# antopio26/quadruped-gym

Hardware: AMD Instinct MI355X
Metric: env_steps_per_sec (higher is better)
Workload: dtype f32

## Files before the change

### quadruped-gym_amd/csrc/qg_kernel_link.hip

```cpp
#define QGK_LINK_ENVS 4
#include "qg_po_dev.h"

typedef const __attribute__((address_space(1))) char *lk_gcbytes;
typedef __attribute__((address_space(1))) char *lk_gbytes;
template <class T> DEV T lk_ld(const T *base, unsigned byte_off) { return *(const __attribute__((address_space(1))) T *)((lk_gcbytes)base + byte_off); }
template <class T> DEV void lk_st(T *base, unsigned byte_off, T v) { *(__attribute__((address_space(1))) T *)((lk_gbytes)base + byte_off) = v; }

template <int CTRL> DEV float dpp_any(float x) {
    return __builtin_bit_cast(float, __builtin_amdgcn_mov_dpp(__builtin_bit_cast(int, x), CTRL, 0xF, 0xF, true));
}
DEV float env_sum(float x) {
#pragma clang fp contract(off)
    x += dpp_any<0xB1>(x);
    x += dpp_any<0x4E>(x);
    x += dpp_any<0x141>(x);
    x += dpp_any<0x140>(x);
    return x;
}
DEV V3 env_sum(V3 a) { return v3(env_sum(a.x), env_sum(a.y), env_sum(a.z)); }
#define QG_T_HM(d, s, bm) "v_add_f32_dpp %[" d "], %[" s "], %[" s "] row_half_mirror row_mask:0xf bank_mask:" bm "\n\t"
#define QG_T_ROR(d, s, bm) "v_add_f32_dpp %[" d "], %[" s "], %[" s "] row_ror:8 row_mask:0xf bank_mask:" bm "\n\t"
#define QG_T_QP(d, qp) "v_add_f32_dpp %[" d "], %[" d "], %[" d "] quad_perm:" qp " row_mask:0xf bank_mask:0xf\n\t"
#define QG_T_L1(g) QG_T_HM("a" g, "a" g, "0x5") QG_T_HM("c" g, "c" g, "0x5") QG_T_HM("a" g, "b" g, "0xa") QG_T_HM("c" g, "d" g, "0xa")
#define QG_T_L2(g) QG_T_ROR("a" g, "a" g, "0x3") QG_T_ROR("a" g, "c" g, "0xc")
#define QG_T_Q1(g) QG_T_QP("a" g, "[1,0,3,2]")
#define QG_T_Q2(g) QG_T_QP("a" g, "[2,3,0,1]")
#define QG_T_OUT(g, v) [a##g] "+v"(v[4 * g]), [c##g] "+v"(v[4 * g + 2])
#define QG_T_IN(g, v) [b##g] "v"(v[4 * g + 1]), [d##g] "v"(v[4 * g + 3])
DEV void env_sum_banked16(float (&v)[16]) {
    asm("s_nop 1\n\t" QG_T_L1("0") QG_T_L1("1") QG_T_L1("2") QG_T_L1("3") QG_T_L2("0") QG_T_L2("1") QG_T_L2("2") QG_T_L2("3")
        QG_T_Q1("0") QG_T_Q1("1") QG_T_Q1("2") QG_T_Q1("3") QG_T_Q2("0") QG_T_Q2("1") QG_T_Q2("2") QG_T_Q2("3") "s_nop 1"
        : QG_T_OUT(0, v), QG_T_OUT(1, v), QG_T_OUT(2, v), QG_T_OUT(3, v)
        : QG_T_IN(0, v), QG_T_IN(1, v), QG_T_IN(2, v), QG_T_IN(3, v));
}
DEV void env_sum_banked12(float (&v)[12]) {
    asm("s_nop 1\n\t" QG_T_L1("0") QG_T_L1("1") QG_T_L1("2") QG_T_L2("0") QG_T_L2("1") QG_T_L2("2")
        QG_T_Q1("0") QG_T_Q1("1") QG_T_Q1("2") QG_T_Q2("0") QG_T_Q2("1") QG_T_Q2("2") "s_nop 1"
        : QG_T_OUT(0, v), QG_T_OUT(1, v), QG_T_OUT(2, v)
        : QG_T_IN(0, v), QG_T_IN(1, v), QG_T_IN(2, v));
}
template <int K> DEV float banked_sum(float r) { return dpp_any<0x150 + 4 * K>(r); }
DEV float leg_suffix(float x) {
#pragma clang fp contract(off)
    x += dpp_any<0xF9>(x);
    x += dpp_any<0xFE>(x);
    return x;
}
#define QG_Z_FM(i) "v_fmac_f32_dpp %[z" i "], %[z" i "], %[c] quad_perm:[1,1,1,1] row_mask:0xf bank_mask:0xf\n\t"
DEV float leg_bcast0(float x) { return dpp_any<0x00>(x); }
DEV float leg_bcast1(float x) { return dpp_any<0x55>(x); }
DEV float leg_bcast2(float x) { return dpp_any<0xAA>(x); }

DEV float leg_prefix(float x) {
#pragma clang fp contract(off)
    x += dpp_any<0xD3>(x);
    x += dpp_any<0x4F>(x);
    return x;
}
DEV V3 leg_prefix(V3 a) { return v3(leg_prefix(a.x), leg_prefix(a.y), leg_prefix(a.z)); }

struct LinkRegs {
    float mass, ipos[3], inertia[6], cp[QGK_CP_LINK][3];
    f2 cp2[QGK_CP_LINK / 2][3];
    float lo, hi, damping, armature, kp, kv, gear, force_lo, force_hi, act_decay;
    float cpF[3];
    float ml;
    float fb[8];
};
struct HingeLane { float q, qd, act, u, sn, cs; };
struct KXfrcLink { KWrench w; V3 c0; };

DEV float sel3(int r, float a, float b, float c) { return r == 0 ? a : (r == 1 ? b : c); }
DEV V3 sel3(int r, V3 a, V3 b, V3 c) { return v3(sel3(r, a.x, b.x, c.x), sel3(r, a.y, b.y, c.y), sel3(r, a.z, b.z, c.z)); }

template <bool BAKED, bool DYN = false>
DEV void substep_link(const KModel &C, float cm, float sm, int r, bool lead_env, BaseState &B, HingeLane &J, const LinkRegs &K,
                      bool want_sensors, float *__restrict__ row, int kleg, float &zaxis_z, const KDyn &D = KDyn{}, bool xon = false,
                      const KXfrcLink &X = KXfrcLink{}) {
    using namespace pk3;
    const float h = C.h;
    const BaseCtx bc = pk3::base_prelude_unit<BAKED>(C, B);
    const V3 nb = bc.n;
    if (want_sensors) {
        zaxis_z = bc.cz.z;
        if (r < 3) row[3 * kleg + r] = J.q;
        if (lead_env) {
            row[15] = B.wb.x; row[16] = B.wb.y; row[17] = B.wb.z;
            row[18] = B.pw.x; row[19] = B.pw.y; row[20] = B.pw.z;
            row[21] = B.vw.x; row[22] = B.vw.y; row[23] = B.vw.z;
            row[24] = bc.cx.x; row[25] = bc.cx.y; row[26] = bc.cx.z;
            row[27] = bc.cz.x; row[28] = bc.cz.y; row[29] = bc.cz.z;
            row[30] = bc.vb.x; row[31] = bc.vb.y; row[32] = bc.vb.z;
        }
    }
    const int rr = r < 2 ? r : 2;
    const float snj[3] = {leg_bcast0(J.sn), leg_bcast1(J.sn), leg_bcast2(J.sn)};
    const float csj[3] = {leg_bcast0(J.cs), leg_bcast1(J.cs), leg_bcast2(J.cs)};
    Fr E[3];
    V3 p[3];
    SV S[3];
    {
        Fr Ep = {v3(BAKED ? cm : 1.f, BAKED ? sm : 0.f, 0.f), v3(BAKED ? -sm : 0.f, BAKED ? cm : 1.f, 0.f), v3(0.f, 0.f, 1.f)};
        V3 pp = v3(0.f, 0.f, 0.f);
#pragma unroll
        for (int i = 0; i < 3; ++i) {
            const KLink &L = link_of<BAKED>(C, kleg, i);
            const float sn = snj[i], cs = csj[i];
            p[i] = pp + rot(Ep, ld3(L.pos));
            V3 tx = fma3(L.Q[0], Ep.ex, fma3(L.Q[3], Ep.ey, L.Q[6] * Ep.ez));
            V3 ty = fma3(L.Q[1], Ep.ex, fma3(L.Q[4], Ep.ey, L.Q[7] * Ep.ez));
            V3 tz = fma3(L.Q[2], Ep.ex, fma3(L.Q[5], Ep.ey, L.Q[8] * Ep.ez));
            E[i].ex = fma3(cs, tx, sn * ty);
            E[i].ey = fma3(cs, ty, (-sn) * tx);
            E[i].ez = tz;
            S[i].a = E[i].ez;
            S[i].l = cross(p[i], E[i].ez);
            Ep = E[i]; pp = p[i];
        }
    }
    const Fr Ep = {sel3(rr, E[0].ex, E[1].ex, E[2].ex), sel3(rr, E[0].ey, E[1].ey, E[2].ey), sel3(rr, E[0].ez, E[1].ez, E[2].ez)};
    const V3 pp = sel3(rr, p[0], p[1], p[2]);
    const SV So = {Ep.ez, cross(pp, Ep.ez)};
    SV vp, ap;
    {
        const float qdm = K.ml * J.qd;
        const SV Sq = {qdm * So.a, qdm * So.l};
        vp.a = leg_prefix(Sq.a) + bc.V0.a;
        vp.l = leg_prefix(Sq.l) + bc.V0.l;
        const V3 ca = cross(vp.a, Sq.a);
        const V3 cl = cross_add(vp.l, Sq.a, cross(vp.a, Sq.l));
        ap.a = leg_prefix(ca) + bc.A0.a;
        ap.l = leg_prefix(cl) + bc.A0.l;
    }
    Rigid Bi;
    Bi.m = K.mass;
    V3 cl;
    {
        const Fr &E = Ep;
        V3 c = pp + rot(E, v3(K.ipos[0], K.ipos[1], K.ipos[2]));
        cl = c;
        Bi.h = Bi.m * c;
        V3 ux = fma3(K.inertia[0], E.ex, fma3(K.inertia[3], E.ey, K.inertia[4] * E.ez));
        V3 uy = fma3(K.inertia[3], E.ex, fma3(K.inertia[1], E.ey, K.inertia[5] * E.ez));
        V3 uz = fma3(K.inertia[4], E.ex, fma3(K.inertia[5], E.ey, K.inertia[2] * E.ez));
        float hc = dot(Bi.h, c);
        const f2 uxp = {ux.x, ux.y}, uyp = {uy.x, uy.y}, uzp = {uz.x, uz.y}, hp = {Bi.h.x, Bi.h.y}, cp2 = {c.x, c.y};
        const f2 d2 = __builtin_elementwise_fma(uxp, f2{E.ex.x, E.ex.y}, __builtin_elementwise_fma(uyp, f2{E.ey.x, E.ey.y}, uzp * f2{E.ez.x, E.ez.y}))
                      + f2{hc, hc} - hp * cp2;
        const f2 o2 = __builtin_elementwise_fma(uxp, f2{E.ex.z, E.ex.z}, __builtin_elementwise_fma(uyp, f2{E.ey.z, E.ey.z}, uzp * f2{E.ez.z, E.ez.z}))
                      - hp * f2{c.z, c.z};
        Bi.I.xx = d2.x; Bi.I.yy = d2.y; Bi.I.xz = o2.x; Bi.I.yz = o2.y;
        Bi.I.zz = fmaf(ux.z, E.ex.z, fmaf(uy.z, E.ey.z, uz.z * E.ez.z)) + hc - Bi.h.z * c.z;
        Bi.I.xy = fmaf(ux.x, E.ex.y, fmaf(uy.x, E.ey.y, uz.x * E.ez.y)) - Bi.h.x * c.y;
    }
    SV f;
    {
        SV Iv = mul(Bi, vp), Ia = mul(Bi, ap);
        f.a = cross_add(vp.l, Iv.l, cross_add(vp.a, Iv.a, Ia.a));
        f.l = cross_add(vp.a, Iv.l, Ia.l);
    }
    Sym6 A = sym6_of(Bi);
    {
        const float zo = B.pw.z + dot(nb, pp);
        V3 nl = rotT(Ep, nb);
        float wsum = 0.f;
        V3 s = v3(0.f, 0.f, 0.f);
        const float zb = C.contact_margin - zo;
        if constexpr (BAKED) {
            static_assert(QGK_CP_LINK % 2 == 0, "sample points are taken in pairs");
            f2 w2 = {0.f, 0.f};
            V3T<f2> s2 = v3<f2>(w2, w2, w2);
            const V3T<f2> nl2 = v3<f2>(f2{nl.x, nl.x}, f2{nl.y, nl.y}, f2{nl.z, nl.z});
            const f2 zb2 = {zb, zb};
#pragma unroll
            for (int i = 0; i < QGK_CP_LINK / 2; ++i) contact_point(v3<f2>(K.cp2[i][0], K.cp2[i][1], K.cp2[i][2]), nl2, zb2, w2, s2);
            wsum = w2.x + w2.y;
            s = v3(opaque(s2.x.x + s2.x.y), opaque(s2.y.x + s2.y.y), s2.z.x + s2.z.y);
        } else {
#pragma unroll
            for (int i = 0; i < QGK_CP_LINK; ++i) contact_point(v3(K.cp[i][0], K.cp[i][1], K.cp[i][2]), nl, zb, wsum, s);
        }
        wsum *= K.ml;
        SV fe;
        ContactDampT<float> cd;
        if constexpr (DYN) pk3::contact_eval(wsum, s, Ep, pp, nb, vp, D.kc, D.cc, C.contact_inv_ramp, D.mu, h, fe, cd);
        else pk3::contact_eval(wsum, s, Ep, pp, nb, vp, C.contact_k, C.contact_c, C.contact_inv_ramp, C.contact_mu, h, fe, cd);
        f.a = f.a - fe.a;
        f.l = f.l - fe.l;
        if constexpr (BAKED) pk3::add_contact_damping<true>(A, cd.mc, cd.w, cd.P, nb, Bi.h);
        else pk3::add_contact_damping(A, cd.mc, cd.w, cd.P, nb);
    }
    SV xw = {};
    if constexpr (DYN) {
        if (xon) {
            xw = xfrc_spatial(bc, X.w, r < 3 ? cl : X.c0);
            f.a = fma3(-K.ml, xw.a, f.a);
            f.l = fma3(-K.ml, xw.l, f.l);
        }
    }
    float wsumF = 0.f;
    V3 sF = v3(0.f, 0.f, 0.f);
    contact_point(v3(K.cpF[0], K.cpF[1], K.cpF[2]), nb, C.contact_margin - B.pw.z, wsumF, sF);
    wsumF *= K.ml; sF = K.ml * sF;
    Sym6 Ic;
    SV fc;
    Ic.AA.xx = leg_suffix(A.AA.xx); Ic.AA.yy = leg_suffix(A.AA.yy); Ic.AA.zz = leg_suffix(A.AA.zz);
    Ic.AA.xy = leg_suffix(A.AA.xy); Ic.AA.xz = leg_suffix(A.AA.xz); Ic.AA.yz = leg_suffix(A.AA.yz);
    Ic.AL.r0 = v3(leg_suffix(A.AL.r0.x), leg_suffix(A.AL.r0.y), leg_suffix(A.AL.r0.z));
    Ic.AL.r1 = v3(leg_suffix(A.AL.r1.x), leg_suffix(A.AL.r1.y), leg_suffix(A.AL.r1.z));
    Ic.AL.r2 = v3(leg_suffix(A.AL.r2.x), leg_suffix(A.AL.r2.y), leg_suffix(A.AL.r2.z));
    Ic.LL.xx = leg_suffix(A.LL.xx); Ic.LL.yy = leg_suffix(A.LL.yy); Ic.LL.zz = leg_suffix(A.LL.zz);
    Ic.LL.xy = leg_suffix(A.LL.xy); Ic.LL.xz = leg_suffix(A.LL.xz); Ic.LL.yz = leg_suffix(A.LL.yz);
    fc.a = v3(leg_suffix(f.a.x), leg_suffix(f.a.y), leg_suffix(f.a.z));
    fc.l = v3(leg_suffix(f.l.x), leg_suffix(f.l.y), leg_suffix(f.l.z));
    const SV F = mul(Ic, So);
    const float Hc0 = dot(S[0], F), Hc1 = dot(S[1], F);
    const float Hown = dot(So, F);
    const float tb = dot(So, fc);
    float Hd_o, b_o;
    {
        const float q = J.q, qd = J.qd, act = J.act;
        float force = K.kp * (act - K.gear * q) - (K.kv * K.gear) * qd;
        const bool clamped = force <= K.force_lo || force >= K.force_hi;
        force = fminf(fmaxf(force, K.force_lo), K.force_hi);
        float dimp = K.damping + (clamped ? 0.f : K.kv * K.gear * K.gear);
        float tau = K.gear * force - K.damping * qd;
        const float below = K.lo - q, above = q - K.hi;
        const float pen = fmaxf(fmaxf(below, above), 0.f);
        const float bl = C.limit_b * fminf(pen * C.limit_inv_ramp, 1.f);
        const float sg = below > above ? 1.f : -1.f;
        const float sqd = sg * qd;
        const float spring = C.limit_k * pen;
        const float tq = spring - bl * sqd;
        const bool leaving = tq < 0.f;
        tau = fmaf(sg, fmaxf(tq, 0.f), tau);
        dimp = dimp + (leaving ? spring * rcp(sqd) : bl);
        Hd_o = Hown + K.armature + h * dimp;
        b_o = tau - tb;
    }
    const float H00 = leg_bcast0(Hd_o), H01 = leg_bcast1(Hc0), H11 = leg_bcast1(Hd_o);
    const float H02 = leg_bcast2(Hc0), H12 = leg_bcast2(Hc1), H22 = leg_bcast2(Hd_o);
    const float b0 = leg_bcast0(b_o), b1 = leg_bcast1(b_o), b2 = leg_bcast2(b_o);
    const float id0 = rcp(H00);
    const float l10 = H01 * id0, l20 = H02 * id0;
    const float d1 = fmaf(-l10, H01, H11), id1 = rcp(d1);
    const float t21 = fmaf(-l20, H01, H12);
    const float l21 = t21 * id1;
    const float d2 = fmaf(-l21, t21, fmaf(-l20, H02, H22)), id2 = rcp(d2);
    const float y0 = b0, y1 = fmaf(-l10, y0, b1), y2 = fmaf(-l21, y1, fmaf(-l20, y0, b2));
    float z[6] = {F.a.x, F.a.y, F.a.z, F.l.x, F.l.y, F.l.z};
    {
        const float nc0 = r == 1 ? -l10 : (r == 2 ? -l20 : 0.f), nc1 = r == 2 ? -l21 : 0.f;
#pragma unroll
        for (int i = 0; i < 6; ++i) z[i] = fmaf(leg_bcast0(z[i]), nc0, z[i]);
        if constexpr (BAKED) {
            asm("s_nop 1\n\t" QG_Z_FM("0") QG_Z_FM("1") QG_Z_FM("2") QG_Z_FM("3") QG_Z_FM("4") QG_Z_FM("5")
                : [z0] "+v"(z[0]), [z1] "+v"(z[1]), [z2] "+v"(z[2]), [z3] "+v"(z[3]), [z4] "+v"(z[4]), [z5] "+v"(z[5])
                : [c] "v"(nc1));
        } else {
#pragma unroll
            for (int i = 0; i < 6; ++i) z[i] = fmaf(leg_bcast1(z[i]), nc1, z[i]);
        }
    }
    const float idr = sel3(rr, id0, id1, id2), yr = sel3(rr, y0, y1, y2);
    const f2 P = {z[0], z[1]}, L = {z[3], z[4]}, Z = {z[2], z[5]};
    const f2 idr2 = {idr, idr};
    const f2 WP = idr2 * P, WL = idr2 * L, WZ = idr2 * Z;
    Sym6 Cn;
    {
        const f2 Zlo = {Z.x, Z.x}, Zhi = {Z.y, Z.y};
        const f2 WPlo = {WP.x, WP.x}, WPhi = {WP.y, WP.y}, WZlo = {WZ.x, WZ.x};
        const f2 aa0 = __builtin_elementwise_fma(-WP, P, f2{A.AA.xx, A.AA.yy});
        const f2 aa1 = __builtin_elementwise_fma(-WP, Zlo, f2{A.AA.xz, A.AA.yz});
        Cn.AA.xx = aa0.x; Cn.AA.yy = aa0.y; Cn.AA.xz = aa1.x; Cn.AA.yz = aa1.y;
        Cn.AA.xy = fmaf(-WP.x, P.y, A.AA.xy); Cn.AA.zz = fmaf(-WZ.x, Z.x, A.AA.zz);
        const f2 c0 = __builtin_elementwise_fma(-WPlo, L, f2{A.AL.r0.x, A.AL.r0.y});
        const f2 c1 = __builtin_elementwise_fma(-WPhi, L, f2{A.AL.r1.x, A.AL.r1.y});
        const f2 c2 = __builtin_elementwise_fma(-WZlo, L, f2{A.AL.r2.x, A.AL.r2.y});
        const f2 c3 = __builtin_elementwise_fma(-WP, Zhi, f2{A.AL.r0.z, A.AL.r1.z});
        Cn.AL.r0 = v3(c0.x, c0.y, c3.x);
        Cn.AL.r1 = v3(c1.x, c1.y, c3.y);
        Cn.AL.r2 = v3(c2.x, c2.y, fmaf(-WZ.x, Z.y, A.AL.r2.z));
        const f2 l0 = __builtin_elementwise_fma(-WL, L, f2{A.LL.xx, A.LL.yy});
        const f2 l1 = __builtin_elementwise_fma(-WL, Zhi, f2{A.LL.xz, A.LL.yz});
        Cn.LL.xx = l0.x; Cn.LL.yy = l0.y; Cn.LL.xz = l1.x; Cn.LL.yz = l1.y;
        Cn.LL.xy = fmaf(-WL.x, L.y, A.LL.xy); Cn.LL.zz = fmaf(-WZ.y, Z.y, A.LL.zz);
    }
    if constexpr (DYN) {
        if (xon) {
            f.a = fma3(K.ml - 1.f, xw.a, f.a);
            f.l = fma3(K.ml - 1.f, xw.l, f.l);
        }
    }
    const f2 nyr = {-yr, -yr};
    const f2 rh0 = __builtin_elementwise_fma(nyr, WP, f2{-f.a.x, -f.a.y}), rh1 = __builtin_elementwise_fma(nyr, WL, f2{-f.l.x, -f.l.y}),
             rh2 = BAKED ? __builtin_elementwise_fma(nyr, WZ, -f2{f.a.z, f.l.z})
                         : __builtin_elementwise_fma(nyr, WZ, f2{-f.a.z, -f.l.z});
    SV rhn = {v3(rh0.x, rh0.y, rh2.x), v3(rh1.x, rh1.y, rh2.y)};
    float x6[6];
    {
        SV p0;
        Sym6 Ic0;
        pk3::frame_body_pk<DYN>(C, bc, h, p0, Ic0, D);
        if constexpr (BAKED) {
            Ic0.AA.xx = K.fb[0]; Ic0.AA.yy = K.fb[1]; Ic0.AA.zz = K.fb[2]; Ic0.LL.xx = K.fb[3]; Ic0.LL.yy = K.fb[4]; Ic0.LL.zz = K.fb[5];
            Ic0.AL.r0.y = K.fb[6]; Ic0.AL.r1.x = K.fb[7];
        }
        float t16[16] = {Cn.AA.xx, Cn.AA.yy, Cn.AA.zz, Cn.AA.xy, Cn.AA.xz, Cn.AA.yz, Cn.AL.r0.x, Cn.AL.r0.y,
                         Cn.AL.r0.z, Cn.AL.r1.x, Cn.AL.r1.y, Cn.AL.r1.z, Cn.AL.r2.x, Cn.AL.r2.y, Cn.AL.r2.z, wsumF};
        float t12[12] = {Cn.LL.xx, Cn.LL.yy, Cn.LL.zz, Cn.LL.xy, Cn.LL.xz, Cn.LL.yz, rhn.a.x, rhn.a.y, rhn.a.z, rhn.l.x, rhn.l.y, rhn.l.z};
        env_sum_banked16(t16);
        env_sum_banked12(t12);
        Ic0.AA.xx += banked_sum<0>(t16[0]); Ic0.AA.yy += banked_sum<1>(t16[0]); Ic0.AA.zz += banked_sum<2>(t16[0]); Ic0.AA.xy += banked_sum<3>(t16[0]);
        Ic0.AA.xz += banked_sum<0>(t16[4]); Ic0.AA.yz += banked_sum<1>(t16[4]); Ic0.AL.r0.x += banked_sum<2>(t16[4]); Ic0.AL.r0.y += banked_sum<3>(t16[4]);
        Ic0.AL.r0.z += banked_sum<0>(t16[8]); Ic0.AL.r1.x += banked_sum<1>(t16[8]); Ic0.AL.r1.y += banked_sum<2>(t16[8]); Ic0.AL.r1.z += banked_sum<3>(t16[8]);
        Ic0.AL.r2.x += banked_sum<0>(t16[12]); Ic0.AL.r2.y += banked_sum<1>(t16[12]); Ic0.AL.r2.z += banked_sum<2>(t16[12]);
        wsumF = banked_sum<3>(t16[12]);
        Ic0.LL.xx += banked_sum<0>(t12[0]); Ic0.LL.yy += banked_sum<1>(t12[0]); Ic0.LL.zz += banked_sum<2>(t12[0]); Ic0.LL.xy += banked_sum<3>(t12[0]);
        Ic0.LL.xz += banked_sum<0>(t12[4]); Ic0.LL.yz += banked_sum<1>(t12[4]);
        SV b = {v3(banked_sum<2>(t12[4]) - p0.a.x, banked_sum<3>(t12[4]) - p0.a.y, banked_sum<0>(t12[8]) - p0.a.z),
                v3(banked_sum<1>(t12[8]) - p0.l.x, banked_sum<2>(t12[8]) - p0.l.y, banked_sum<3>(t12[8]) - p0.l.z)};
        if (__any(wsumF > 0.f)) {
            sF = env_sum(sF);
            Fr E0 = {v3(1.f, 0.f, 0.f), v3(0.f, 1.f, 0.f), v3(0.f, 0.f, 1.f)};
            SV fe;
            if constexpr (DYN) contact_finish(wsumF, sF, E0, v3(0.f, 0.f, 0.f), bc.n, bc.V0, D.kc, D.cc, C.contact_inv_ramp, D.mu, h, fe, Ic0);
            else contact_finish(wsumF, sF, E0, v3(0.f, 0.f, 0.f), bc.n, bc.V0, C.contact_k, C.contact_c, C.contact_inv_ramp, C.contact_mu, h, fe, Ic0);
            b.a = b.a + fe.a;
            b.l = b.l + fe.l;
        }
        pk3::base_solve(Ic0, b, x6);
    }
    const V3 wdot = v3(x6[0], x6[1], x6[2]);
    const V3 acl = v3(x6[3], x6[4], x6[5]);
    if (want_sensors && lead_env) {
        row[12] = acl.x - bc.gb.x; row[13] = acl.y - bc.gb.y; row[14] = acl.z - bc.gb.z;
    }
    {
        const float g_o = fmaf(F.a.x, x6[0], fmaf(F.a.y, x6[1], fmaf(F.a.z, x6[2], fmaf(F.l.x, x6[3], fmaf(F.l.y, x6[4], F.l.z * x6[5])))));
        const float r0 = b0 - leg_bcast0(g_o), r1 = b1 - leg_bcast1(g_o), r2 = b2 - leg_bcast2(g_o);
        const float yy0 = r0, yy1 = fmaf(-l10, yy0, r1), yy2 = fmaf(-l21, yy1, fmaf(-l20, yy0, r2));
        const float qdd2 = yy2 * id2;
        const float qdd1 = fmaf(-l21, qdd2, yy1 * id1);
        const float qdd0 = fmaf(-l20, qdd2, fmaf(-l10, qdd1, yy0 * id0));
        J.qd = fmaf(h, sel3(rr, qdd0, qdd1, qdd2), J.qd);
        J.q = fmaf(h, J.qd, J.q);
        hinge_advance(h * J.qd, J.sn, J.cs);
        J.act = fmaf(J.u - J.act, K.act_decay, J.act);
    }
    pk3::base_integrate_unit<BAKED>(bc, h, wdot, acl, B);
}

#define QGK_LINK_WAVES 4
template <bool WALK = false, bool PO = false, bool BAKED = true, bool HELP = false, bool DYN = false>
__global__ __launch_bounds__(QGK_WAVE * QGK_LINK_WAVES * (HELP ? 2 : 1), 1) void qg_step_kernel_link(const KModel *__restrict__ Mp, const KTask *__restrict__ T, KStepArgs P,
                                                                                  const typename WalkArgT<WALK>::type WK,
                                                                                  const typename PoArgT<PO>::type PK) {
    static_assert(WALK || !PO, "the observation pack rides on the walking task layer");
    static_assert(WALK || !HELP, "the helper waves carry the walking task layer's estimator");
    static_assert(!DYN || (!BAKED && !HELP), "per-env dynamics: the table-driven variants");
    static_assert(QGK_LINK_ENVS * QGK_LINK_WAVES == QG_PO_ENVS && QGK_WAVE * QGK_LINK_WAVES == QG_PO_THREADS, "workgroup layout of qg_po_dev.h");
    __shared__ float tile_all[QGK_LINK_WAVES][QGK_LINK_ENVS * 35];
    __shared__ KModel smodel;
    QG_STAGE_MODEL(C, BAKED, smodel, Mp, QGK_WAVE * QGK_LINK_WAVES * (HELP ? 2 : 1));
    QG_TASK_REGS(Tk, T);
// ... 302 lines not shown
```

### quadruped-gym_amd/csrc/qg_kernels.hip

```cpp
#include <hip/hip_runtime.h>
#include <stdint.h>

#include "qg_device.h"
#include "qg_model_baked.h"
#include "qg_step_shell.h"

#define DEV __device__ __forceinline__
#define QG_STR2(x) #x
#define QG_STR(x) QG_STR2(x)

static __device__ const KModel QG_BAKED_MODEL = {QG_BAKED_FLOATS};
template <bool BAKED> DEV const KModel &table(const KModel *__restrict__ M) {
    if constexpr (BAKED) return QG_BAKED_MODEL; else return *M;
}
template <bool BAKED> DEV const KLink &link_of(const KModel &C, int k, int i) { return C.link[BAKED ? i : 3 * k + i]; }

typedef float f2 __attribute__((ext_vector_type(2)));
typedef int i2 __attribute__((ext_vector_type(2)));

DEV float fma_(float a, float b, float c) { return fmaf(a, b, c); }
DEV f2 fma_(f2 a, f2 b, f2 c) { return __builtin_elementwise_fma(a, b, c); }
DEV float max_(float a, float b) { return fmaxf(a, b); }
DEV f2 max_(f2 a, f2 b) { f2 r = {fmaxf(a.x, b.x), fmaxf(a.y, b.y)}; return r; }
DEV float min_(float a, float b) { return fminf(a, b); }
// ... 5 lines not shown
DEV float sqrt_(float x) { return __builtin_amdgcn_sqrtf(x); }
DEV f2 sqrt_(f2 x) { f2 r = {__builtin_amdgcn_sqrtf(x.x), __builtin_amdgcn_sqrtf(x.y)}; return r; }
DEV float sel(bool m, float a, float b) { return m ? a : b; }
DEV f2 sel(i2 m, f2 a, f2 b) { f2 r = {m.x ? a.x : b.x, m.y ? a.y : b.y}; return r; }
DEV bool m_and(bool a, bool b) { return a && b; }
DEV i2 m_and(i2 a, i2 b) { return a & b; }
DEV bool m_or(bool a, bool b) { return a || b; }
DEV i2 m_or(i2 a, i2 b) { return a | b; }
DEV bool m_not(bool a) { return !a; }
DEV i2 m_not(i2 a) { return ~a; }
DEV bool m_any(bool a) { return a; }
DEV bool m_any(i2 a) { return (a.x | a.y) != 0; }
template <class T> DEV T splat(float x) { return T(x); }

template <class T> struct V3T { T x, y, z; };
typedef V3T<float> V3;
template <class T> DEV V3T<T> v3(T x, T y, T z) { V3T<T> r = {x, y, z}; return r; }
template <class T> DEV V3T<T> operator+(V3T<T> a, V3T<T> b) { return v3<T>(a.x + b.x, a.y + b.y, a.z + b.z); }
template <class T> DEV V3T<T> operator-(V3T<T> a, V3T<T> b) { return v3<T>(a.x - b.x, a.y - b.y, a.z - b.z); }
template <class T> DEV V3T<T> operator*(T s, V3T<T> a) { return v3<T>(s * a.x, s * a.y, s * a.z); }
template <class T> DEV T dot(V3T<T> a, V3T<T> b) { return fma_(a.x, b.x, fma_(a.y, b.y, a.z * b.z)); }
template <class T> DEV V3T<T> cross(V3T<T> a, V3T<T> b) { return v3<T>(a.y * b.z - a.z * b.y, a.z * b.x - a.x * b.z, a.x * b.y - a.y * b.x); }
template <class T> DEV V3T<T> fma3(T s, V3T<T> a, V3T<T> b) { return v3<T>(fma_(s, a.x, b.x), fma_(s, a.y, b.y), fma_(s, a.z, b.z)); }
namespace pk3 {
DEV V3 fma3(float s, V3 a, V3 b) { f2 A = {a.x, a.y}, Bv = {b.x, b.y}, S = {s, s}; f2 r = __builtin_elementwise_fma(S, A, Bv); return v3<float>(r.x, r.y, fmaf(s, a.z, b.z)); }
DEV V3 operator+(V3 a, V3 b) { f2 A = {a.x, a.y}, Bv = {b.x, b.y}; f2 r = A + Bv; return v3<float>(r.x, r.y, a.z + b.z); }
DEV V3 operator-(V3 a, V3 b) { f2 A = {a.x, a.y}, Bv = {b.x, b.y}; f2 r = A - Bv; return v3<float>(r.x, r.y, a.z - b.z); }
DEV V3 operator*(float s, V3 a) { f2 A = {a.x, a.y}, S = {s, s}; f2 r = S * A; return v3<float>(r.x, r.y, s * a.z); }
DEV bool has_literal(V3 a) { return __builtin_constant_p(a.x) || __builtin_constant_p(a.y) || __builtin_constant_p(a.z); }
DEV V3 cross(V3 a, V3 b) {
    if (has_literal(a) || has_literal(b)) return ::cross<float>(a, b);
    f2 A = {a.x, a.y}, Bv = {b.x, b.y}, az, bz, m, r;
    az.x = a.z; bz.x = b.z;
    asm("v_pk_mul_f32 %0, %1, %2 op_sel:[0,1] op_sel_hi:[0,0] neg_lo:[1,0]" : "=v"(m) : "v"(az), "v"(Bv));
    asm("v_pk_fma_f32 %0, %1, %2, %3 op_sel:[1,0,0] op_sel_hi:[0,0,1] neg_hi:[1,0,0]" : "=v"(r) : "v"(A), "v"(bz), "v"(m));
    return v3<float>(r.x, r.y, a.x * b.y - a.y * b.x);
}
DEV V3 cross_add(V3 a, V3 b, V3 acc) {
    if (has_literal(a) || has_literal(b)) return ::operator+<float>(acc, ::cross<float>(a, b));
    f2 A = {a.x, a.y}, Bv = {b.x, b.y}, C2 = {acc.x, acc.y}, az, bz, m, r;
    az.x = a.z; bz.x = b.z;
    asm("v_pk_fma_f32 %0, %1, %2, %3 op_sel:[0,1,0] op_sel_hi:[0,0,1] neg_lo:[1,0,0]" : "=v"(m) : "v"(az), "v"(Bv), "v"(C2));
    asm("v_pk_fma_f32 %0, %1, %2, %3 op_sel:[1,0,0] op_sel_hi:[0,0,1] neg_hi:[1,0,0]" : "=v"(r) : "v"(A), "v"(bz), "v"(m));
    return v3<float>(r.x, r.y, fmaf(a.x, b.y, fmaf(-a.y, b.x, acc.z)));
}
DEV V3 cross_sub(V3 a, V3 b, V3 acc) {
    if (has_literal(a) || has_literal(b)) return cross_add(a, b, v3<float>(-acc.x, -acc.y, -acc.z));
    f2 A = {a.x, a.y}, Bv = {b.x, b.y}, C2 = {acc.x, acc.y}, az, bz, m, r;
    az.x = a.z; bz.x = b.z;
    asm("v_pk_fma_f32 %0, %1, %2, %3 op_sel:[0,1,0] op_sel_hi:[0,0,1] neg_lo:[1,0,1] neg_hi:[0,0,1]" : "=v"(m) : "v"(az), "v"(Bv), "v"(C2));
    asm("v_pk_fma_f32 %0, %1, %2, %3 op_sel:[1,0,0] op_sel_hi:[0,0,1] neg_hi:[1,0,0]" : "=v"(r) : "v"(A), "v"(bz), "v"(m));
    return v3<float>(r.x, r.y, fmaf(a.x, b.y, fmaf(-a.y, b.x, -acc.z)));
}
}
DEV V3 ld3(const float *p) { return v3<float>(p[0], p[1], p[2]); }
template <class T> DEV V3T<T> ld3t(const float *p) { return v3<T>(T(p[0]), T(p[1]), T(p[2])); }
template <class T> DEV V3T<T> splat3(V3 a) { return v3<T>(T(a.x), T(a.y), T(a.z)); }

template <class T> struct FrT { V3T<T> ex, ey, ez; };
typedef FrT<float> Fr;
template <class T> DEV V3T<T> rot(const FrT<T> &E, V3T<T> r) { return fma3(r.x, E.ex, fma3(r.y, E.ey, r.z * E.ez)); }
template <class T> DEV V3T<T> rotT(const FrT<T> &E, V3T<T> r) { return v3<T>(dot(E.ex, r), dot(E.ey, r), dot(E.ez, r)); }

template <class T> struct Sym3T { T xx, yy, zz, xy, xz, yz; };
typedef Sym3T<float> Sym3;
template <class T> DEV V3T<T> mul(const Sym3T<T> &S, V3T<T> v) {
    return v3<T>(fma_(S.xx, v.x, fma_(S.xy, v.y, S.xz * v.z)), fma_(S.xy, v.x, fma_(S.yy, v.y, S.yz * v.z)),
                 fma_(S.xz, v.x, fma_(S.yz, v.y, S.zz * v.z)));
}
template <class T> DEV void add(Sym3T<T> &a, const Sym3T<T> &b) { a.xx += b.xx; a.yy += b.yy; a.zz += b.zz; a.xy += b.xy; a.xz += b.xz; a.yz += b.yz; }
template <class T> DEV void rank1(Sym3T<T> &a, T w, V3T<T> u, V3T<T> v) {
    a.xx = fma_(w * u.x, v.x, a.xx); a.yy = fma_(w * u.y, v.y, a.yy); a.zz = fma_(w * u.z, v.z, a.zz);
    a.xy = fma_(w * u.x, v.y, a.xy); a.xz = fma_(w * u.x, v.z, a.xz); a.yz = fma_(w * u.y, v.z, a.yz);
}

template <class T> struct M3T { V3T<T> r0, r1, r2; };
typedef M3T<float> M3;
template <class T> DEV V3T<T> mul(const M3T<T> &A, V3T<T> v) { return v3<T>(dot(A.r0, v), dot(A.r1, v), dot(A.r2, v)); }
template <class T> DEV V3T<T> mulT(const M3T<T> &A, V3T<T> v) { return fma3(v.x, A.r0, fma3(v.y, A.r1, v.z * A.r2)); }
template <class T> DEV void add(M3T<T> &a, const M3T<T> &b) { a.r0 = a.r0 + b.r0; a.r1 = a.r1 + b.r1; a.r2 = a.r2 + b.r2; }

template <class T> struct SVT { V3T<T> a, l; };
typedef SVT<float> SV;
template <class T> DEV SVT<T> operator+(SVT<T> p, SVT<T> q) { SVT<T> r = {p.a + q.a, p.l + q.l}; return r; }
template <class T> DEV T dot(SVT<T> p, SVT<T> q) { return dot(p.a, q.a) + dot(p.l, q.l); }
template <class T> DEV SVT<T> splat6(SV v) { SVT<T> r = {splat3<T>(v.a), splat3<T>(v.l)}; return r; }

template <class T> struct RigidT { T m; V3T<T> h; Sym3T<T> I; };
typedef RigidT<float> Rigid;
template <class T> DEV SVT<T> mul(const RigidT<T> &B, SVT<T> v) {
    SVT<T> f;
    f.a = mul(B.I, v.a) + cross(B.h, v.l);
    f.l = B.m * v.l - cross(B.h, v.a);
    return f;
}

template <class T> struct Sym6T { Sym3T<T> AA; M3T<T> AL; Sym3T<T> LL; };
typedef Sym6T<float> Sym6;
template <class T> DEV SVT<T> mul(const Sym6T<T> &A, SVT<T> s) {
    SVT<T> f;
    f.a = mul(A.AA, s.a) + mul(A.AL, s.l);
    f.l = mulT(A.AL, s.a) + mul(A.LL, s.l);
    return f;
}
template <class T> DEV void add(Sym6T<T> &a, const Sym6T<T> &b) { add(a.AA, b.AA); add(a.AL, b.AL); add(a.LL, b.LL); }
namespace pk3 {
DEV float dot(SV p, SV q) {
    if (has_literal(p.a) || has_literal(p.l) || has_literal(q.a) || has_literal(q.l)) return ::dot<float>(p, q);
    const f2 t = __builtin_elementwise_fma(f2{p.l.x, p.l.y}, f2{q.l.x, q.l.y}, f2{p.a.x, p.a.y} * f2{q.a.x, q.a.y});
    return fmaf(p.l.z, q.l.z, fmaf(p.a.z, q.a.z, t.x)) + t.y;
}
DEV f2 fma_swapped(float s, f2 v, f2 acc) {
    f2 sp, r;
    sp.x = s;
    asm("v_pk_fma_f32 %0, %1, %2, %3 op_sel:[0,1,0] op_sel_hi:[0,0,1]" : "=v"(r) : "v"(sp), "v"(v), "v"(acc));
    return r;
}
DEV V3 mul(const Sym3 &S, V3 v) {
    const f2 d = {S.xx, S.yy}, o = {S.xz, S.yz}, vxy = {v.x, v.y}, vz = {v.z, v.z};
    const f2 r = __builtin_elementwise_fma(d, vxy, fma_swapped(S.xy, vxy, o * vz));
    return v3<float>(r.x, r.y, fmaf(S.xz, v.x, fmaf(S.yz, v.y, S.zz * v.z)));
}
DEV V3 mulT(const M3 &A, V3 v) { return fma3(v.x, A.r0, fma3(v.y, A.r1, v.z * A.r2)); }
DEV V3 rot(const Fr &E, V3 r) { return fma3(r.x, E.ex, fma3(r.y, E.ey, r.z * E.ez)); }
DEV SV mul(const Rigid &B, SV v) {
    SV f;
    f.a = cross_add(B.h, v.l, mul(B.I, v.a));
    f.l = cross_add(v.a, B.h, B.m * v.l);
    return f;
}
DEV SV mul(const Sym6 &A, SV s) {
    SV f;
    f.a = mul(A.AA, s.a) + ::mul(A.AL, s.l);
    f.l = mulT(A.AL, s.a) + mul(A.LL, s.l);
    return f;
}
}
template <class T> DEV Sym6T<T> sym6_of(const RigidT<T> &B) {
    Sym6T<T> A;
    const T z = T(0.f);
    A.AA = B.I;
    A.AL.r0 = v3<T>(z, -B.h.z, B.h.y);
    A.AL.r1 = v3<T>(B.h.z, z, -B.h.x);
    A.AL.r2 = v3<T>(-B.h.y, B.h.x, z);
    A.LL.xx = A.LL.yy = A.LL.zz = B.m;
    A.LL.xy = A.LL.xz = A.LL.yz = z;
    return A;
}
template <class T> DEV void add_contact_damping(Sym6T<T> &A, T m, T w, V3T<T> r, V3T<T> n) {
    T rr = dot(r, r);
    A.AA.xx += m * (rr - r.x * r.x); A.AA.yy += m * (rr - r.y * r.y); A.AA.zz += m * (rr - r.z * r.z);
    A.AA.xy -= m * r.x * r.y; A.AA.xz -= m * r.x * r.z; A.AA.yz -= m * r.y * r.z;
    V3T<T> h = m * r;
    const T z = T(0.f);
    A.AL.r0 = A.AL.r0 + v3<T>(z, -h.z, h.y);
    A.AL.r1 = A.AL.r1 + v3<T>(h.z, z, -h.x);
    A.AL.r2 = A.AL.r2 + v3<T>(-h.y, h.x, z);
    A.LL.xx += m; A.LL.yy += m; A.LL.zz += m;
    V3T<T> ra = cross(r, n);
    rank1(A.AA, w, ra, ra);
    A.AL.r0 = fma3(w * ra.x, n, A.AL.r0);
    A.AL.r1 = fma3(w * ra.y, n, A.AL.r1);
    A.AL.r2 = fma3(w * ra.z, n, A.AL.r2);
    rank1(A.LL, w, n, n);
}

DEV void sincos_quadrant(float k, float sr, float cr, float &s, float &c) {
    int q = (int)k;
    float s0 = (q & 1) ? cr : sr;
    float c0 = (q & 1) ? sr : cr;
    s = (q & 2) ? -s0 : s0;
    c = ((q + 1) & 2) ? -c0 : c0;
}
DEV float rint_(float x) { return rintf(x); }
DEV f2 rint_(f2 x) { f2 r = {rintf(x.x), rintf(x.y)}; return r; }
template <class T> DEV void sincos_f(T x, T &s, T &c) {
    T k = rint_(x * 0.63661977236758134f);
    T r = fma_(-k, T(1.57079625129699707031f), x);
    r = fma_(-k, T(7.54978941586159635335e-08f), r);
    T r2 = r * r;
    T sp = fma_(r2, fma_(r2, fma_(r2, T(2.718311493989822e-06f), T(-1.984090162742e-04f)), T(8.333329385889463e-03f)), T(-1.666666597127914e-01f));
    T sr = fma_(r * r2, sp, r);
    T cp = fma_(r2, fma_(r2, fma_(r2, T(2.443315711809948e-05f), T(-1.388731625493765e-03f)), T(4.166664568298827e-02f)), T(-0.5f));
    T cr = fma_(r2, cp, T(1.0f));
    if constexpr (sizeof(T) == sizeof(float)) {
        sincos_quadrant(k, sr, cr, s, c);
    } else {
        float s0, c0, s1, c1;
// ... 1717 lines not shown
```

### quadruped-gym_amd/csrc/qg_link_regs.inc

```
    LinkRegs K;
    {
        const int rk = r < 2 ? r : 2;
        const KLink &L0 = C.link[0], &L1 = C.link[1], &L2 = C.link[2];
        const KLink &Lown = C.link[3 * k + rk];
        const float ml = r < 3 ? 1.f : 0.f;
        const float s0 = rk == 0 ? 1.f : 0.f, s1 = rk == 1 ? 1.f : 0.f, s2 = rk == 2 ? 1.f : 0.f;
#define QG_SEL(field) (BAKED ? ((L0.field == L1.field && L1.field == L2.field) ? L0.field \
                                                                               : fmaf(s2, L2.field, fmaf(s1, L1.field, s0 * L0.field))) \
                             : Lown.field)
        K.mass = ml * QG_SEL(mass);
#pragma unroll
        for (int i = 0; i < 3; ++i) K.ipos[i] = QG_SEL(ipos[i]);
#pragma unroll
        for (int i = 0; i < 6; ++i) K.inertia[i] = ml * QG_SEL(inertia[i]);
#pragma unroll
        for (int i = 0; i < QGK_CP_LINK; ++i) { K.cp[i][0] = QG_SEL(cp[i][0]); K.cp[i][1] = QG_SEL(cp[i][1]); K.cp[i][2] = QG_SEL(cp[i][2]); }
#pragma unroll
        for (int i = 0; i < QGK_CP_LINK / 2; ++i)
#pragma unroll
            for (int c = 0; c < 3; ++c) K.cp2[i][c] = f2{K.cp[i][c], K.cp[i + QGK_CP_LINK / 2][c]};
        K.lo = QG_SEL(lo); K.hi = QG_SEL(hi); K.damping = QG_SEL(damping); K.armature = QG_SEL(armature); K.kp = QG_SEL(kp);
        K.kv = QG_SEL(kv); K.gear = QG_SEL(gear); K.force_lo = QG_SEL(force_lo); K.force_hi = QG_SEL(force_hi);
        K.act_decay = QG_SEL(act_decay);
        K.ml = ml;
        if constexpr (BAKED) {
            const float fx = sel3(rk, C.cp0[0][0], C.cp0[4][0], C.cp0[8][0]), fy = sel3(rk, C.cp0[0][1], C.cp0[4][1], C.cp0[8][1]);
            K.cpF[0] = cm * fx - sm * fy; K.cpF[1] = sm * fx + cm * fy; K.cpF[2] = sel3(rk, C.cp0[0][2], C.cp0[4][2], C.cp0[8][2]);
        } else {
            K.cpF[0] = C.cp0[3 * k + rk][0]; K.cpF[1] = C.cp0[3 * k + rk][1]; K.cpF[2] = C.cp0[3 * k + rk][2];
        }
#undef QG_SEL
        if constexpr (BAKED) {
            const float dg = C.free_armature + C.h * C.free_damping;
            K.fb[0] = pk3::opaque(C.I0[0] + dg); K.fb[1] = pk3::opaque(C.I0[1] + dg); K.fb[2] = pk3::opaque(C.I0[2] + dg);
            K.fb[3] = pk3::opaque(C.m0 + dg); K.fb[4] = pk3::opaque(C.m0 + dg); K.fb[5] = pk3::opaque(C.m0 + dg);
            K.fb[6] = pk3::opaque(-C.h0[2]); K.fb[7] = pk3::opaque(C.h0[2]);
        }
    }
```

Before: 428.1 million.

## Pack z-components into packed-FP32 ops and fold identity mount link

Rewrites the per-link spatial cross products, rigid/Sym6 multiplies and inertia rotation in the baked path so their z components are paired and issued as v_pk_mul/v_pk_fma instructions. When the third link's mount rotation is the identity, the kinematic chain selection collapses to two candidates by zeroing the middle link's contribution. The two banked DPP environment reductions are merged into one asm block to share the surrounding nops. The aim is fewer VALU instructions per substep, in exchange for extra packed register state (iz) and inline asm that constrains scheduling.

```diff
diff --git a/quadruped-gym_amd/csrc/qg_kernel_link.hip b/quadruped-gym_amd/csrc/qg_kernel_link.hip
--- a/quadruped-gym_amd/csrc/qg_kernel_link.hip
+++ b/quadruped-gym_amd/csrc/qg_kernel_link.hip
@@ -27,17 +27,15 @@
 #define QG_T_Q2(g) QG_T_QP("a" g, "[2,3,0,1]")
 #define QG_T_OUT(g, v) [a##g] "+v"(v[4 * g]), [c##g] "+v"(v[4 * g + 2])
 #define QG_T_IN(g, v) [b##g] "v"(v[4 * g + 1]), [d##g] "v"(v[4 * g + 3])
-DEV void env_sum_banked16(float (&v)[16]) {
-    asm("s_nop 1\n\t" QG_T_L1("0") QG_T_L1("1") QG_T_L1("2") QG_T_L1("3") QG_T_L2("0") QG_T_L2("1") QG_T_L2("2") QG_T_L2("3")
-        QG_T_Q1("0") QG_T_Q1("1") QG_T_Q1("2") QG_T_Q1("3") QG_T_Q2("0") QG_T_Q2("1") QG_T_Q2("2") QG_T_Q2("3") "s_nop 1"
-        : QG_T_OUT(0, v), QG_T_OUT(1, v), QG_T_OUT(2, v), QG_T_OUT(3, v)
-        : QG_T_IN(0, v), QG_T_IN(1, v), QG_T_IN(2, v), QG_T_IN(3, v));
-}
-DEV void env_sum_banked12(float (&v)[12]) {
-    asm("s_nop 1\n\t" QG_T_L1("0") QG_T_L1("1") QG_T_L1("2") QG_T_L2("0") QG_T_L2("1") QG_T_L2("2")
-        QG_T_Q1("0") QG_T_Q1("1") QG_T_Q1("2") QG_T_Q2("0") QG_T_Q2("1") QG_T_Q2("2") "s_nop 1"
-        : QG_T_OUT(0, v), QG_T_OUT(1, v), QG_T_OUT(2, v)
-        : QG_T_IN(0, v), QG_T_IN(1, v), QG_T_IN(2, v));
+#define QG_T_OUT2(g, h, w) [a##g] "+v"(w[4 * h]), [c##g] "+v"(w[4 * h + 2])
+#define QG_T_IN2(g, h, w) [b##g] "v"(w[4 * h + 1]), [d##g] "v"(w[4 * h + 3])
+DEV void env_sum_banked28(float (&v)[16], float (&w)[12]) {
+    asm("s_nop 1\n\t" QG_T_L1("0") QG_T_L1("1") QG_T_L1("2") QG_T_L1("3") QG_T_L1("4") QG_T_L1("5") QG_T_L1("6")
+        QG_T_L2("0") QG_T_L2("1") QG_T_L2("2") QG_T_L2("3") QG_T_L2("4") QG_T_L2("5") QG_T_L2("6")
+        QG_T_Q1("0") QG_T_Q1("1") QG_T_Q1("2") QG_T_Q1("3") QG_T_Q1("4") QG_T_Q1("5") QG_T_Q1("6")
+        QG_T_Q2("0") QG_T_Q2("1") QG_T_Q2("2") QG_T_Q2("3") QG_T_Q2("4") QG_T_Q2("5") QG_T_Q2("6") "s_nop 1"
+        : QG_T_OUT(0, v), QG_T_OUT(1, v), QG_T_OUT(2, v), QG_T_OUT(3, v), QG_T_OUT2(4, 0, w), QG_T_OUT2(5, 1, w), QG_T_OUT2(6, 2, w)
+        : QG_T_IN(0, v), QG_T_IN(1, v), QG_T_IN(2, v), QG_T_IN(3, v), QG_T_IN2(4, 0, w), QG_T_IN2(5, 1, w), QG_T_IN2(6, 2, w));
 }
 template <int K> DEV float banked_sum(float r) { return dpp_any<0x150 + 4 * K>(r); }
 DEV float leg_suffix(float x) {
@@ -66,12 +64,17 @@
     float cpF[3];
     float ml;
     float fb[8];
+    f2 iz[2][3];
 };
 struct HingeLane { float q, qd, act, u, sn, cs; };
 struct KXfrcLink { KWrench w; V3 c0; };
 
 DEV float sel3(int r, float a, float b, float c) { return r == 0 ? a : (r == 1 ? b : c); }
 DEV V3 sel3(int r, V3 a, V3 b, V3 c) { return v3(sel3(r, a.x, b.x, c.x), sel3(r, a.y, b.y, c.y), sel3(r, a.z, b.z, c.z)); }
+DEV V3 sel2(int r, V3 a, V3 b) { return v3(r == 0 ? a.x : b.x, r == 0 ? a.y : b.y, r == 0 ? a.z : b.z); }
+DEV bool mount_is_identity(const float *Q) {
+    return Q[0] == 1.f && Q[1] == 0.f && Q[2] == 0.f && Q[3] == 0.f && Q[4] == 1.f && Q[5] == 0.f && Q[6] == 0.f && Q[7] == 0.f && Q[8] == 1.f;
+}
 
 template <bool BAKED, bool DYN = false>
 DEV void substep_link(const KModel &C, float cm, float sm, int r, bool lead_env, BaseState &B, HingeLane &J, const LinkRegs &K,
@@ -99,14 +102,21 @@
     Fr E[3];
     V3 p[3];
     SV S[3];
+    const bool fold2 = BAKED && mount_is_identity(link_of<BAKED>(C, kleg, 2).Q);
     {
         Fr Ep = {v3(BAKED ? cm : 1.f, BAKED ? sm : 0.f, 0.f), v3(BAKED ? -sm : 0.f, BAKED ? cm : 1.f, 0.f), v3(0.f, 0.f, 1.f)};
         V3 pp = v3(0.f, 0.f, 0.f);
 #pragma unroll
         for (int i = 0; i < 3; ++i) {
             const KLink &L = link_of<BAKED>(C, kleg, i);
-            const float sn = snj[i], cs = csj[i];
-            p[i] = pp + rot(Ep, ld3(L.pos));
+            float sn = snj[i], cs = csj[i];
+            V3 lp = ld3(L.pos);
+            if (fold2 && i == 2) {
+                const bool own = rr == 2;
+                sn = own ? sn : 0.f; cs = own ? cs : 1.f;
+                lp = v3(own ? lp.x : 0.f, own ? lp.y : 0.f, own ? lp.z : 0.f);
+            }
+            p[i] = pp + rot(Ep, lp);
             V3 tx = fma3(L.Q[0], Ep.ex, fma3(L.Q[3], Ep.ey, L.Q[6] * Ep.ez));
             V3 ty = fma3(L.Q[1], Ep.ex, fma3(L.Q[4], Ep.ey, L.Q[7] * Ep.ez));
             V3 tz = fma3(L.Q[2], Ep.ex, fma3(L.Q[5], Ep.ey, L.Q[8] * Ep.ez));
@@ -118,17 +128,25 @@
             Ep = E[i]; pp = p[i];
         }
     }
-    const Fr Ep = {sel3(rr, E[0].ex, E[1].ex, E[2].ex), sel3(rr, E[0].ey, E[1].ey, E[2].ey), sel3(rr, E[0].ez, E[1].ez, E[2].ez)};
-    const V3 pp = sel3(rr, p[0], p[1], p[2]);
+    const Fr Ep = fold2 ? Fr{sel2(rr, E[0].ex, E[2].ex), sel2(rr, E[0].ey, E[2].ey), sel2(rr, E[0].ez, E[2].ez)}
+                        : Fr{sel3(rr, E[0].ex, E[1].ex, E[2].ex), sel3(rr, E[0].ey, E[1].ey, E[2].ey), sel3(rr, E[0].ez, E[1].ez, E[2].ez)};
+    const V3 pp = fold2 ? sel2(rr, p[0], p[2]) : sel3(rr, p[0], p[1], p[2]);
     const SV So = {Ep.ez, cross(pp, Ep.ez)};
     SV vp, ap;
     {
         const float qdm = K.ml * J.qd;
-        const SV Sq = {qdm * So.a, qdm * So.l};
+        const SV Sq = BAKED ? sv_scale(qdm, So) : SV{qdm * So.a, qdm * So.l};
         vp.a = leg_prefix(Sq.a) + bc.V0.a;
         vp.l = leg_prefix(Sq.l) + bc.V0.l;
-        const V3 ca = cross(vp.a, Sq.a);
-        const V3 cl = cross_add(vp.l, Sq.a, cross(vp.a, Sq.l));
+        V3 ca, cl;
+        if constexpr (BAKED) {
+            const f2 vz = zp(vp), qz = zp(Sq);
+            ca = cross_zp<0, 0>(vp.a, vz, Sq.a, qz);
+            cl = cross_add_zp<1, 0>(vp.l, vz, Sq.a, qz, cross_zp<0, 1>(vp.a, vz, Sq.l, qz));
+        } else {
+            ca = cross(vp.a, Sq.a);
+            cl = cross_add(vp.l, Sq.a, cross(vp.a, Sq.l));
+        }
         ap.a = leg_prefix(ca) + bc.A0.a;
         ap.l = leg_prefix(cl) + bc.A0.l;
     }
@@ -138,11 +156,18 @@
     {
         const Fr &E = Ep;
         V3 c = pp + rot(E, v3(K.ipos[0], K.ipos[1], K.ipos[2]));
-        cl = c;
-        Bi.h = Bi.m * c;
         V3 ux = fma3(K.inertia[0], E.ex, fma3(K.inertia[3], E.ey, K.inertia[4] * E.ez));
         V3 uy = fma3(K.inertia[3], E.ex, fma3(K.inertia[1], E.ey, K.inertia[5] * E.ez));
         V3 uz = fma3(K.inertia[4], E.ex, fma3(K.inertia[5], E.ey, K.inertia[2] * E.ez));
+        if constexpr (BAKED) {
+            const f2 exz = {E.ex.z, E.ex.z}, eyz = {E.ey.z, E.ey.z}, ezz = {E.ez.z, E.ez.z};
+            const f2 z01 = __builtin_elementwise_fma(K.iz[0][0], exz, __builtin_elementwise_fma(K.iz[0][1], eyz, K.iz[0][2] * ezz));
+            const f2 z2c = __builtin_elementwise_fma(K.iz[1][0], exz, __builtin_elementwise_fma(K.iz[1][1], eyz, K.iz[1][2] * ezz));
+            ux.z = z01.x; uy.z = z01.y; uz.z = z2c.x;
+            c.z = pp.z + z2c.y;
+        }
+        cl = c;
+        Bi.h = Bi.m * c;
         float hc = dot(Bi.h, c);
         const f2 uxp = {ux.x, ux.y}, uyp = {uy.x, uy.y}, uzp = {uz.x, uz.y}, hp = {Bi.h.x, Bi.h.y}, cp2 = {c.x, c.y};
         const f2 d2 = __builtin_elementwise_fma(uxp, f2{E.ex.x, E.ex.y}, __builtin_elementwise_fma(uyp, f2{E.ey.x, E.ey.y}, uzp * f2{E.ez.x, E.ez.y}))
@@ -154,7 +179,12 @@
         Bi.I.xy = fmaf(ux.x, E.ex.y, fmaf(uy.x, E.ey.y, uz.x * E.ez.y)) - Bi.h.x * c.y;
     }
     SV f;
-    {
+    if constexpr (BAKED) {
+        const SV Iv = mul_zp(Bi, vp), Ia = mul_zp(Bi, ap);
+        const f2 vz = zp(vp), iz = zp(Iv);
+        f.a = cross_add_zp<1, 1>(vp.l, vz, Iv.l, iz, cross_add_zp<0, 0>(vp.a, vz, Iv.a, iz, Ia.a));
+        f.l = cross_add_zp<0, 1>(vp.a, vz, Iv.l, iz, Ia.l);
+    } else {
         SV Iv = mul(Bi, vp), Ia = mul(Bi, ap);
         f.a = cross_add(vp.l, Iv.l, cross_add(vp.a, Iv.a, Ia.a));
         f.l = cross_add(vp.a, Iv.l, Ia.l);
@@ -213,7 +243,7 @@
     Ic.LL.xy = leg_suffix(A.LL.xy); Ic.LL.xz = leg_suffix(A.LL.xz); Ic.LL.yz = leg_suffix(A.LL.yz);
     fc.a = v3(leg_suffix(f.a.x), leg_suffix(f.a.y), leg_suffix(f.a.z));
     fc.l = v3(leg_suffix(f.l.x), leg_suffix(f.l.y), leg_suffix(f.l.z));
-    const SV F = mul(Ic, So);
+    const SV F = BAKED ? mul_zp(Ic, So) : mul(Ic, So);
     const float Hc0 = dot(S[0], F), Hc1 = dot(S[1], F);
     const float Hown = dot(So, F);
     const float tb = dot(So, fc);
@@ -309,8 +339,7 @@
         float t16[16] = {Cn.AA.xx, Cn.AA.yy, Cn.AA.zz, Cn.AA.xy, Cn.AA.xz, Cn.AA.yz, Cn.AL.r0.x, Cn.AL.r0.y,
                          Cn.AL.r0.z, Cn.AL.r1.x, Cn.AL.r1.y, Cn.AL.r1.z, Cn.AL.r2.x, Cn.AL.r2.y, Cn.AL.r2.z, wsumF};
         float t12[12] = {Cn.LL.xx, Cn.LL.yy, Cn.LL.zz, Cn.LL.xy, Cn.LL.xz, Cn.LL.yz, rhn.a.x, rhn.a.y, rhn.a.z, rhn.l.x, rhn.l.y, rhn.l.z};
-        env_sum_banked16(t16);
-        env_sum_banked12(t12);
+        env_sum_banked28(t16, t12);
         Ic0.AA.xx += banked_sum<0>(t16[0]); Ic0.AA.yy += banked_sum<1>(t16[0]); Ic0.AA.zz += banked_sum<2>(t16[0]); Ic0.AA.xy += banked_sum<3>(t16[0]);
         Ic0.AA.xz += banked_sum<0>(t16[4]); Ic0.AA.yz += banked_sum<1>(t16[4]); Ic0.AL.r0.x += banked_sum<2>(t16[4]); Ic0.AL.r0.y += banked_sum<3>(t16[4]);
         Ic0.AL.r0.z += banked_sum<0>(t16[8]); Ic0.AL.r1.x += banked_sum<1>(t16[8]); Ic0.AL.r1.y += banked_sum<2>(t16[8]); Ic0.AL.r1.z += banked_sum<3>(t16[8]);
diff --git a/quadruped-gym_amd/csrc/qg_kernels.hip b/quadruped-gym_amd/csrc/qg_kernels.hip
--- a/quadruped-gym_amd/csrc/qg_kernels.hip
+++ b/quadruped-gym_amd/csrc/qg_kernels.hip
@@ -81,6 +81,30 @@
     asm("v_pk_fma_f32 %0, %1, %2, %3 op_sel:[1,0,0] op_sel_hi:[0,0,1] neg_hi:[1,0,0]" : "=v"(r) : "v"(A), "v"(bz), "v"(m));
     return v3<float>(r.x, r.y, fmaf(a.x, b.y, fmaf(-a.y, b.x, -acc.z)));
 }
+DEV f2 lone(float z) { f2 p; p.x = z; return p; }
+#define QG_CROSS_MUL(m, az, Bv, AH) \
+    asm("v_pk_mul_f32 %0, %1, %2 op_sel:[" #AH ",1] op_sel_hi:[" #AH ",0] neg_lo:[1,0]" : "=v"(m) : "v"(az), "v"(Bv))
+#define QG_CROSS_MAD(m, az, Bv, C2, AH) \
+    asm("v_pk_fma_f32 %0, %1, %2, %3 op_sel:[" #AH ",1,0] op_sel_hi:[" #AH ",0,1] neg_lo:[1,0,0]" : "=v"(m) : "v"(az), "v"(Bv), "v"(C2))
+#define QG_CROSS_FMA(r, A, bz, m, BH) \
+    asm("v_pk_fma_f32 %0, %1, %2, %3 op_sel:[1," #BH ",0] op_sel_hi:[0," #BH ",1] neg_hi:[1,0,0]" : "=v"(r) : "v"(A), "v"(bz), "v"(m))
+template <int AH, int BH> DEV V3 cross_zp(V3 a, f2 az, V3 b, f2 bz) {
+    const f2 A = {a.x, a.y}, Bv = {b.x, b.y};
+    f2 m, r;
+    if constexpr (AH == 0) QG_CROSS_MUL(m, az, Bv, 0); else QG_CROSS_MUL(m, az, Bv, 1);
+    if constexpr (BH == 0) QG_CROSS_FMA(r, A, bz, m, 0); else QG_CROSS_FMA(r, A, bz, m, 1);
+    return v3<float>(r.x, r.y, a.x * b.y - a.y * b.x);
+}
+template <int AH, int BH> DEV V3 cross_add_zp(V3 a, f2 az, V3 b, f2 bz, V3 acc) {
+    const f2 A = {a.x, a.y}, Bv = {b.x, b.y}, C2 = {acc.x, acc.y};
+    f2 m, r;
+    if constexpr (AH == 0) QG_CROSS_MAD(m, az, Bv, C2, 0); else QG_CROSS_MAD(m, az, Bv, C2, 1);
+    if constexpr (BH == 0) QG_CROSS_FMA(r, A, bz, m, 0); else QG_CROSS_FMA(r, A, bz, m, 1);
+    return v3<float>(r.x, r.y, fmaf(a.x, b.y, fmaf(-a.y, b.x, acc.z)));
+}
+#undef QG_CROSS_MUL
+#undef QG_CROSS_MAD
+#undef QG_CROSS_FMA
 }
 DEV V3 ld3(const float *p) { return v3<float>(p[0], p[1], p[2]); }
 template <class T> DEV V3T<T> ld3t(const float *p) { return v3<T>(T(p[0]), T(p[1]), T(p[2])); }
@@ -163,6 +187,39 @@
     f.a = mul(A.AA, s.a) + ::mul(A.AL, s.l);
     f.l = mulT(A.AL, s.a) + mul(A.LL, s.l);
     return f;
+}
+DEV f2 zp(SV v) { return f2{v.a.z, v.l.z}; }
+DEV SV sv_scale(float s, SV v) {
+    const f2 S = {s, s}, a = S * f2{v.a.x, v.a.y}, l = S * f2{v.l.x, v.l.y}, z = S * f2{v.a.z, v.l.z};
+    return SV{v3<float>(a.x, a.y, z.x), v3<float>(l.x, l.y, z.y)};
+}
+DEV f2 mul_bhi(f2 a, f2 b) { f2 r; asm("v_pk_mul_f32 %0, %1, %2 op_sel:[0,1] op_sel_hi:[1,1]" : "=v"(r) : "v"(a), "v"(b)); return r; }
+DEV SV mul_zp(const Rigid &B, SV v) {
+    const f2 vz = zp(v), va = {v.a.x, v.a.y};
+    const f2 t = f2{B.I.zz, B.m} * vz;
+    const f2 r = __builtin_elementwise_fma(f2{B.I.xx, B.I.yy}, va, fma_swapped(B.I.xy, va, f2{B.I.xz, B.I.yz} * f2{vz.x, vz.x}));
+    const f2 ml = f2{B.m, B.m} * f2{v.l.x, v.l.y};
+    const f2 hz = lone(B.h.z);
+    SV f;
+    f.a = cross_add_zp<0, 1>(B.h, hz, v.l, vz, v3<float>(r.x, r.y, fmaf(B.I.xz, v.a.x, fmaf(B.I.yz, v.a.y, t.x))));
+    f.l = cross_add_zp<0, 0>(v.a, vz, B.h, hz, v3<float>(ml.x, ml.y, t.y));
+    return f;
+}
+DEV SV mul_zp(const Sym6 &A, SV s) {
+    const f2 sz = zp(s), sa = {s.a.x, s.a.y}, sl = {s.l.x, s.l.y};
+    const f2 t1 = f2{A.AA.zz, A.LL.zz} * sz;
+    f2 t2;
+    asm("v_pk_mul_f32 %0, %1, %2 op_sel:[0,1] op_sel_hi:[0,0]" : "=v"(t2) : "v"(lone(A.AL.r2.z)), "v"(sz));
+    const f2 ra = __builtin_elementwise_fma(f2{A.AA.xx, A.AA.yy}, sa, fma_swapped(A.AA.xy, sa, f2{A.AA.xz, A.AA.yz} * f2{sz.x, sz.x}));
+    const f2 rl = __builtin_elementwise_fma(f2{A.LL.xx, A.LL.yy}, sl, fma_swapped(A.LL.xy, sl, mul_bhi(f2{A.LL.xz, A.LL.yz}, sz)));
+    const f2 m1 = {::dot<float>(A.AL.r0, s.l), ::dot<float>(A.AL.r1, s.l)};
+    const f2 tl = __builtin_elementwise_fma(f2{s.a.x, s.a.x}, f2{A.AL.r0.x, A.AL.r0.y},
+                                            __builtin_elementwise_fma(f2{s.a.y, s.a.y}, f2{A.AL.r1.x, A.AL.r1.y}, f2{sz.x, sz.x} * f2{A.AL.r2.x, A.AL.r2.y}));
+    const f2 fa = ra + m1, fl = tl + rl;
+    const f2 z0 = {fmaf(A.AA.xz, s.a.x, fmaf(A.AA.yz, s.a.y, t1.x)), fmaf(A.LL.xz, s.l.x, fmaf(A.LL.yz, s.l.y, t1.y))};
+    const f2 z1 = {fmaf(A.AL.r2.x, s.l.x, fmaf(A.AL.r2.y, s.l.y, t2.x)), fmaf(s.a.x, A.AL.r0.z, fmaf(s.a.y, A.AL.r1.z, t2.y))};
+    const f2 fz = z0 + z1;
+    return SV{v3<float>(fa.x, fa.y, fz.x), v3<float>(fl.x, fl.y, fz.y)};
 }
 }
 template <class T> DEV Sym6T<T> sym6_of(const RigidT<T> &B) {
diff --git a/quadruped-gym_amd/csrc/qg_link_regs.inc b/quadruped-gym_amd/csrc/qg_link_regs.inc
--- a/quadruped-gym_amd/csrc/qg_link_regs.inc
+++ b/quadruped-gym_amd/csrc/qg_link_regs.inc
@@ -19,6 +19,10 @@
         for (int i = 0; i < QGK_CP_LINK / 2; ++i)
 #pragma unroll
             for (int c = 0; c < 3; ++c) K.cp2[i][c] = f2{K.cp[i][c], K.cp[i + QGK_CP_LINK / 2][c]};
+        if constexpr (BAKED) {
+            K.iz[0][0] = f2{K.inertia[0], K.inertia[3]}; K.iz[0][1] = f2{K.inertia[3], K.inertia[1]}; K.iz[0][2] = f2{K.inertia[4], K.inertia[5]};
+            K.iz[1][0] = f2{K.inertia[4], K.ipos[0]}; K.iz[1][1] = f2{K.inertia[5], K.ipos[1]}; K.iz[1][2] = f2{K.inertia[2], K.ipos[2]};
+        }
         K.lo = QG_SEL(lo); K.hi = QG_SEL(hi); K.damping = QG_SEL(damping); K.armature = QG_SEL(armature); K.kp = QG_SEL(kp);
         K.kv = QG_SEL(kv); K.gear = QG_SEL(gear); K.force_lo = QG_SEL(force_lo); K.force_hi = QG_SEL(force_hi);
         K.act_decay = QG_SEL(act_decay);
```

After: 430.0 million, median of 6. No clear change (+0.4%).
